# GreatDrake/acg-alp-ldpc

Hardware: AMD Instinct MI355X
Metric: decoded frames/sec (+ FER@SNR) for H05.txt 50-iter BP (higher is better)
Workload: dtype f32; 1 GPU; configs[1]: H05.txt 160x280 E=860 sum-product BP, 50 iterations fixed, 1048576 AWGN frames/GPU/step, HBM-resident; frames_per_gpu=1048576, iters=50, early_exit=False, launcher=single process, engine=fused (messages in LDS)

## Files before the change

acg_alp_ldpc_amd/csrc/api.hip:

```cpp
#include <algorithm>
#include <cmath>
#include <cstdio>
#include <cstdlib>
#include <cstring>

#include "handle.hpp"

namespace acg {

static thread_local std::string g_err;
void set_error(const std::string &msg) { g_err = msg; }
const std::string &last_error() { return g_err; }

bool ScatteredAlloc::create(size_t want, size_t chunk_bytes, int dev, bool shuffle, int spread) {
    hipMemAllocationProp prop{};
    prop.type = hipMemAllocationTypePinned;
    prop.location.type = hipMemLocationTypeDevice;
    prop.location.id = dev;
    size_t gran = 0;
    if (hipMemGetAllocationGranularity(&gran, &prop, hipMemAllocationGranularityMinimum) != hipSuccess || gran == 0) return false;
    chunk = (std::max(chunk_bytes, gran) + gran - 1) / gran * gran;
    const size_t n = (want + chunk - 1) / chunk;
    bytes = n * chunk;
    if (hipMemAddressReserve(&va, bytes, 0, nullptr, 0) != hipSuccess) {
// ... 620 lines not shown
            return 0;
        }
        const int algo_b = (d->p.algo == ACG_LDPC_BP_MINSUM) ? 1 : 0;
        for (int mc = 0; mc < 2; mc++) {
            const bool idxreg = !idxlds && c.max_vdeg <= 4 && lay.n_vpass <= 12 && getenv("ACG_BP_NO_IDXREG") == nullptr;
            const bool regular_b = idxreg && c.max_cdeg <= 8 && c.max_vdeg <= 4 && getenv("ACG_BP_NO_REGULAR") == nullptr && is_regular(c);
            const void *kp = bp_block_kernel_ptr(algo_b, d->f64, L, mc != 0, idxlds, idxreg, regular_b);
            if (mc == 0) {
                d->blk_idxlds = idxlds;
                d->blk_idxreg = idxreg;
            }
            if (!kp) {
                set_error("no workgroup-per-frame kernel instance for this configuration");
                return 3;
            }
            if (int rc = bind_kernel(d, mc, kp)) return rc;
        }
        return 0;
    }
    const int fpw = 64 / L;
    const int waves = wp.waves;
    if (waves == 0) {
        if (d->p.engine == ACG_LDPC_ENGINE_AUTO) {
            d->dev_allocs.clear();
            return decoder_setup_streamed(d);
        }
        set_error("frame state does not fit in LDS (160 KiB per CU)");
        return 3;
    }
    d->block = waves * 64;
    d->frames_per_block = waves * fpw;
    d->lds_block = per_frame * fpw * waves + t.idx_lds_bytes;
    const int algo = (d->p.algo == ACG_LDPC_BP_MINSUM) ? 1 : 0;
    const bool sat = !d->p.early_exit && getenv("ACG_BP_NO_SATSKIP") == nullptr;
    d->phi_memo = sat && getenv("ACG_BP_NO_PHIMEMO") == nullptr;
    d->freeze = sat && algo == 0 && !d->f64 && d->maxd <= 8 && idxlds && llr_regs && getenv("ACG_BP_NO_FREEZE") == nullptr;
    d->freeze_gate = getenv("ACG_BP_FREEZE_NO_GATE") == nullptr;
    d->freeze_first = 10;
    d->freeze_period = 1;
    if (const char *e = getenv("ACG_BP_FREEZE_CADENCE")) {
        int f = 0, q = 0;
        if (sscanf(e, "%d,%d", &f, &q) == 2 && f >= 1 && q >= 1 && f < (1 << 12) && q < (1 << 12)) d->freeze_first = f, d->freeze_period = q;
    }
    d->freeze_slot_words = (size_t) lay.a_words + (size_t) BP_MAX_APASS * L;
    for (int mc = 0; mc < 2; mc++) {
        const int variant = wp.variant;
        d->variant = variant;
        const void *kp = bp_kernel_ptr(algo, d->f64, d->maxd, L, mc != 0, variant, sat);
        if (!kp) {
            set_error("no kernel instance for this configuration");
            return 3;
        }
        if (sat && algo == 0 && !d->f64 && d->maxd <= 8 && variant == 2 && getenv("ACG_BP_NO_SPEC") == nullptr) {
            const char *name = nullptr;
            if (const void *ks = bp_spec_kernel_ptr(lay, mc != 0, &name)) {
                kp = ks;
                d->spec = name;
            }
        }
        if (int rc = bind_kernel(d, mc, kp)) return rc;
    }
    return 0;
}

int acg::acg_ldpc_decoder_create_impl(const acg_ldpc_code *code, const acg_ldpc_params *params, acg_ldpc_decoder **out,
                                      hipStream_t on_stream) {
    if (!code || !params || !out) {
        set_error("null argument");
        return 1;
    }
    if (params->max_iter < 0) {
        set_error("max_iter must be >= 0");
        return 1;
    }
    int ndev = 0;
    if (hipGetDeviceCount(&ndev) != hipSuccess || ndev <= 0) {
        set_error("no HIP device available: libacg_ldpc_hip has no CPU fallback");
        return 20;
    }
    DecoderPtr own(new acg_ldpc_decoder());
    acg_ldpc_decoder *d = own.get();
    d->c = code->c;
    d->p = *params;
    int dev = params->device;
    if (dev < 0) {
        if (hipGetDevice(&dev) != hipSuccess) dev = 0;
    }
    if (dev >= ndev) {
        set_error("device ordinal out of range");
        return 1;
    }
    d->device = dev;
    int rc = 0;
    do {
        if (hipSetDevice(dev) != hipSuccess) { set_error("hipSetDevice failed"); rc = 10; break; }
        hipDeviceProp_t prop;
        if (hipGetDeviceProperties(&prop, dev) != hipSuccess) { set_error("hipGetDeviceProperties failed"); rc = 10; break; }
        d->cu_count = prop.multiProcessorCount;
        if (on_stream) {
            d->stream = on_stream;
            d->own_stream = false;
        } else if (hipStreamCreateWithFlags(&d->stream, hipStreamNonBlocking) != hipSuccess) { set_error("hipStreamCreate failed"); rc = 10; break; }
        if (d->counters.reserve(sizeof(unsigned long long) * MC_NCOUNTERS) ||
            d->work_ring.reserve(sizeof(unsigned long long) * acg_ldpc_decoder::WORK_RING)) { set_error("hipMalloc failed"); rc = 10; break; }
        {
            bool evok = true;
            for (int k = 0; k < acg_ldpc_decoder::WORK_RING; k++)
                evok = evok && hipEventCreate(&d->ring_ev0[k]) == hipSuccess && hipEventCreate(&d->ring_ev[k]) == hipSuccess;
            if (!evok) { set_error("hipEventCreate failed"); rc = 10; break; }
        }
// ... 49 lines not shown
    if (grid_blocks) *grid_blocks = d->grid_cap[0];
}

static std::string describe(const acg_ldpc_decoder *d) {
    char b[512];
    const char *algo = d->p.algo == ACG_LDPC_QPADMM ? "qpadmm" : (d->p.algo == ACG_LDPC_BP_MINSUM ? "minsum" : "sum-product");
    int slabs = 0, f32 = 0;
    int64_t slab = 0;
    if (d->admm && admm_device_streamed(d->admm.get(), &slabs, &slab, &f32)) {
        snprintf(b, sizeof b, "%s engine=streamed kernel=admm_streamed_kernel<%s> f64=%d slab_bytes=%lld slabs=%d workspace_bytes=%lld "
                               "workspace=hipMalloc mc_grid=per-point",
                 algo, f32 ? "float" : "double", f32 ? 0 : 1, (long long) slab, slabs, (long long) slab * slabs);
    } else if (d->admm) {
        int lds = 0, L = 0, fpb = 0, grid = 0;
        admm_device_layout(d->admm.get(), &lds, &L, &fpb, &grid);
        snprintf(b, sizeof b, "%s engine=lds lanes_per_frame=%d frames_per_block=%d lds_bytes_per_frame=%d grid_cap=%d mc_grid=%s", algo, L, fpb, lds, grid,
                 admm_device_has_grid_kernel(d->admm.get()) ? "single-launch" : "per-point");
    } else if (d->streamed) {
        const size_t slab = (size_t) d->stab.ws_words_per_wave * 4;
        snprintf(b, sizeof b, "%s engine=streamed kernel=%s%s f64=%d slab_bytes=%zu slabs=%d workspace_bytes=%zu workspace_base=%p "
                               "workgroups_per_cu=%d schedule=%s",
                 algo, d->sring ? "bp_streamed_ring_kernel" : "bp_streamed_kernel", d->sring ? (d->sring_nt ? "<NT>" : "<default-policy>") : "",
                 d->f64, slab, d->sgrid, slab * (size_t) d->sgrid, d->sws.va, d->sring ? d->sring_per_cu : 2,
                 !d->sws.plain ? "flooding workspace=mapped-chunks" : "flooding workspace=hipMalloc");
        if (!d->sws_probe_ms.empty()) {
            std::string t = b;
            t += " workspace_spread=" + std::to_string(d->sws_spread) + " workspace_probe_ms=";
            for (size_t i = 0; i < d->sws_probe_ms.size(); i++) {
                char q[32];
                snprintf(q, sizeof q, "%s%.2f", i ? "/" : "", d->sws_probe_ms[i]);
                t += q;
            }
            return t;
        }
    } else if (d->layered_block) {
        snprintf(b, sizeof b, "%s engine=fused kernel=%s lanes_per_frame=%d f64=0 block=%d frames_per_block=1 lds_block=%zu "
                               "grid_cap=%d sets=%d steps=%d largest_set=%d schedule=layered messages=%s",
                 algo, d->layered_wide ? "bp_layered_wide_kernel" : "bp_layered_block_kernel", d->L, d->block, d->lds_block, d->grid_cap[0], d->lbtab.n_sets, d->lbtab.n_steps, d->lblay.width,
                 d->p.precision == ACG_LDPC_PREC_F16 ? "fp16" : "fp32");
    } else {
        snprintf(b, sizeof b, "%s engine=fused kernel=%s lanes_per_frame=%d f64=%d block=%d frames_per_block=%d lds_block=%zu grid_cap=%d "
                               "idx_lds=%d idx_reg=%d schedule=%s",
                 algo, d->layered ? "bp_layered_kernel" : (d->pair ? "bp_pair_kernel" : (d->variant < 0 ? "bp_block_kernel" : "bp_fused_kernel")), d->L, d->f64, d->block,
                 d->frames_per_block, d->lds_block, d->grid_cap[0], d->variant < 0 ? (int) d->blk_idxlds : (d->variant > 0), (int) d->blk_idxreg,
                 d->p.schedule == ACG_LDPC_SCHEDULE_LAYERED ? (d->p.precision == ACG_LDPC_PREC_F16 ? "layered messages=fp16" : "layered messages=fp32")
                                                            : "flooding");
        if (d->variant >= 0 && !d->layered && !d->pair) {
            std::string t = b;
            if (!d->p.early_exit) {
                if (d->freeze) t += " freeze=1 freeze_cadence=" + std::to_string(d->freeze_first) + "," + std::to_string(d->freeze_period) +
                                        " freeze_gate=" + (d->freeze_gate ? "1" : "0");
                else t += " freeze=0";
            }
            t += std::string(" spec=") + (d->spec ? d->spec : "0");
            return t;
        }
    }
    return b;
}

int32_t acg_ldpc_decoder_describe(const acg_ldpc_decoder *d, char *buf, int32_t cap) {
    if (!d) return 0;
    return copy_text(describe(d), buf, cap);
}

}
```

acg_alp_ldpc_amd/csrc/bp_core.inc:

```


template <typename T> struct FpBits;
template <> struct FpBits<float> {
    using U = uint32_t;
    static constexpr U SIGN = 0x80000000u;
    static __device__ __forceinline__ U to(float x) { return __float_as_uint(x); }
    static __device__ __forceinline__ float from(U u) { return __uint_as_float(u); }
};
template <> struct FpBits<double> {
    using U = uint64_t;
    static constexpr U SIGN = 0x8000000000000000ull;
    static __device__ __forceinline__ U to(double x) { return (U) __double_as_longlong(x); }
    static __device__ __forceinline__ double from(U u) { return __longlong_as_double((long long) u); }
};

__device__ __forceinline__ void wave_sync() {
    __builtin_amdgcn_fence(__ATOMIC_RELEASE, "wavefront");
    __builtin_amdgcn_wave_barrier();
    __builtin_amdgcn_fence(__ATOMIC_ACQUIRE, "wavefront");
}

template <int L>
__device__ __forceinline__ void group_sync() {
    if (L <= 64) wave_sync();
// ... 42 lines not shown
    static constexpr double scale = 1.0;
    static __device__ __forceinline__ double phi(double x) { return phi_f(x); }
};

__device__ __forceinline__ void philox4x32_10(uint32_t c0, uint32_t c1, uint32_t c2, uint32_t c3, uint32_t k0,
                                              uint32_t k1, uint32_t out[4]) {
#pragma unroll
    for (int r = 0; r < 10; ++r) {
        const uint32_t hi0 = __umulhi(0xD2511F53u, c0), lo0 = 0xD2511F53u * c0;
        const uint32_t hi1 = __umulhi(0xCD9E8D57u, c2), lo1 = 0xCD9E8D57u * c2;
        const uint32_t n0 = hi1 ^ c1 ^ k0, n2 = hi0 ^ c3 ^ k1;
        c0 = n0;
        c1 = lo1;
        c2 = n2;
        c3 = lo0;
        k0 += 0x9E3779B9u;
        k1 += 0xBB67AE85u;
    }
    out[0] = c0;
    out[1] = c1;
    out[2] = c2;
    out[3] = c3;
}

__device__ __forceinline__ void box_muller(uint32_t a, uint32_t b, float &z0, float &z1) {
    const float u1 = ((float) a + 0.5f) * 2.3283064365386963e-10f;
    const float u2 = (float) (b >> 8) * 5.9604644775390625e-08f;
    const float r = sqrtf(-2.0f * 0.693147180559945309f * __builtin_amdgcn_logf(u1));
    z0 = r * __builtin_amdgcn_cosf(u2);
    z1 = r * __builtin_amdgcn_sinf(u2);
}

typedef const int32_t __attribute__((address_space(4))) *sconst_i32;
__device__ __forceinline__ int sload(const int32_t *p, int i) { return ((sconst_i32) (p))[i]; }

template <typename T, int D, int L, int ALGO, bool SAT = false>
struct BpPass {
    using B = FpBits<T>;
    using U = typename B::U;
    static constexpr U SIGN = B::SIGN;
    static constexpr U ONE = (U) 1;

    static __device__ __forceinline__ T phi_c(T s, U mb, T G) {
        T o = G;
        if (B::to(s) != mb) o = Dom<T>::phi(s);
        return o;
    }
    static __device__ __forceinline__ T phi_c(T s) { return phi_c(s, (U) 0, (T) INFINITY); }
    static __device__ __forceinline__ T phi_v(T ax) {
        T o = (T) 0;
        if (!(ax >= (T) 66)) o = Dom<T>::phi(ax);
        return o;
    }

    static __device__ __forceinline__ U check_sat(T *__restrict__ Ap, int slot, const int *cnt, bool write) {
        T x[D];
#pragma unroll
        for (int j = 0; j < D; ++j) x[j] = Ap[j * L];
        U S = 0;
#pragma unroll
        for (int j = 0; j < D; ++j) S ^= B::to(x[j]);
        T mag[D], pre[D], es[D];
        T s = 0;
#pragma unroll
        for (int j = 0; j < D; ++j) {
            mag[j] = B::from(B::to(x[j]) & ~SIGN & ~ONE);
            pre[j] = s;
            s += mag[j];
        }
        T suf = 0;
#pragma unroll
        for (int j = D - 1; j >= 0; --j) {
            es[j] = pre[j] + suf;
            suf += mag[j];
        }
#pragma unroll
        for (int j = 0; j < D; ++j) {
            if (write && slot < cnt[j + 1]) {
                const T o = phi_c(es[j]);
                Ap[j * L] = B::from((B::to(o) & ~SIGN) | ((S ^ B::to(x[j])) & SIGN));
            }
        }
        return S;
    }

    static __device__ __forceinline__ U syn(const T *__restrict__ Ap) {
        T x[D];
#pragma unroll
        for (int j = 0; j < D; ++j) x[j] = Ap[j * L];
        U S = 0;
#pragma unroll
        for (int j = 0; j < D; ++j) S ^= B::to(x[j]);
        return S;
    }

    static __device__ __forceinline__ U syn_abs(const T *__restrict__ Ap, U aw) {
        T x[D];
#pragma unroll
        for (int j = 0; j < D - 1; ++j) x[j] = Ap[j * L];
        U S = aw;
#pragma unroll
        for (int j = 0; j < D - 1; ++j) S ^= B::to(x[j]);
        return S;
    }

    template <bool UNI = false>
    static __device__ __forceinline__ U check(T *__restrict__ Ap, int slot, const int *cnt, bool write, T ms_scale) {
        if constexpr (SAT && ALGO == 0 && !UNI) return check_sat(Ap, slot, cnt, write);
        T x[D];
#pragma unroll
        for (int j = 0; j < D; ++j) x[j] = Ap[j * L];
        U S = 0;
#pragma unroll
        for (int j = 0; j < D; ++j) S ^= B::to(x[j]);
        T out[D];
        if (ALGO == 0) {
            T mag[D], pre[D];
            T s = 0;
#pragma unroll
            for (int j = 0; j < D; ++j) {
                mag[j] = B::from(B::to(x[j]) & ~SIGN & ~ONE);
                pre[j] = s;
                s += mag[j];
            }
            T suf = 0;
#pragma unroll
            for (int j = D - 1; j >= 0; --j) {
                out[j] = Dom<T>::phi(pre[j] + suf);
                suf += mag[j];
            }
        } else {
            T m1 = (T) INFINITY, m2 = (T) INFINITY;
            T mag[D];
#pragma unroll
            for (int j = 0; j < D; ++j) {
                const T a0 = B::from(B::to(x[j]) & ~SIGN & ~ONE);
                const T a = (UNI || slot < cnt[j + 1]) ? a0 : (T) INFINITY;
                mag[j] = a;
                if constexpr (sizeof(T) == 4) m2 = __builtin_amdgcn_fmed3f(a, m1, m2);
                else m2 = __builtin_fmin(m2, __builtin_fmax(a, m1));
                m1 = (sizeof(T) == 4) ? (T) __builtin_fminf((float) m1, (float) a) : (T) __builtin_fmin((double) m1, (double) a);
            }
            const T m1s = ms_scale * m1, m2s = ms_scale * m2;
#pragma unroll
            for (int j = 0; j < D; ++j) out[j] = (mag[j] == m1) ? m2s : m1s;
        }
        if (UNI) {
            U obv[D];
#pragma unroll
            for (int j = 0; j < D; ++j) obv[j] = (B::to(out[j]) & ~SIGN) | ((S ^ B::to(x[j])) & SIGN);
            if (write && slot < cnt[D]) {
#pragma unroll
                for (int j = 0; j < D; ++j) Ap[j * L] = B::from(obv[j]);
            }
            return S;
        }
#pragma unroll
        for (int j = 0; j < D; ++j) {
            const U ob = (B::to(out[j]) & ~SIGN) | ((S ^ B::to(x[j])) & SIGN);
            if (write && slot < cnt[j + 1]) Ap[j * L] = B::from(ob);
        }
        return S;
    }

    static __device__ __forceinline__ U check_abs(T *__restrict__ Ap, int slot, const int *cnt, bool write, U &aw, T allr, T &r_out,
                                                  T ag = (T) INFINITY, U am = 0) {
        T x[D];
#pragma unroll
        for (int j = 0; j < D - 1; ++j) x[j] = Ap[j * L];
        x[D - 1] = B::from(aw);
        U S = 0;
#pragma unroll
        for (int j = 0; j < D; ++j) S ^= B::to(x[j]);
        T out[D];
        T mag[D], pre[D];
        T s = 0;
#pragma unroll
        for (int j = 0; j < D; ++j) {
            mag[j] = B::from(B::to(x[j]) & ~SIGN & ~ONE);
            pre[j] = s;
            s += mag[j];
        }
        T suf = 0;
        if constexpr (SAT) {
#pragma unroll
            for (int j = D - 1; j >= 0; --j) {
                out[j] = pre[j] + suf;
                suf += mag[j];
            }
            const U mb = aw & am;
#pragma unroll
            for (int j = 0; j < D - 1; ++j) {
                if (write && slot < cnt[j + 2]) {
                    const T o = phi_c(out[j], mb, ag);
                    Ap[j * L] = B::from((B::to(o) & ~SIGN) | ((S ^ B::to(x[j])) & SIGN));
                }
            }
            if (write && slot < cnt[1]) {
                const T R = B::from((B::to(phi_c(out[D - 1])) & ~SIGN) | ((S ^ aw) & SIGN));
                r_out = R;
                aw = (aw & ~ONE) | ((allr + R <= (T) 0) ? ONE : (U) 0);
            }
            return S;
        }
#pragma unroll
        for (int j = D - 1; j >= 0; --j) {
            out[j] = Dom<T>::phi(pre[j] + suf);
            suf += mag[j];
        }
#pragma unroll
        for (int j = 0; j < D - 1; ++j) {
            const U ob = (B::to(out[j]) & ~SIGN) | ((S ^ B::to(x[j])) & SIGN);
            if (write && slot < cnt[j + 2]) Ap[j * L] = B::from(ob);
        }
        if (write && slot < cnt[1]) {
            const T R = B::from((B::to(out[D - 1]) & ~SIGN) | ((S ^ aw) & SIGN));
            r_out = R;
            aw = (aw & ~ONE) | ((allr + R <= (T) 0) ? ONE : (U) 0);
        }
        return S;
    }

    template <bool BYTES>
    static __device__ __forceinline__ T &at(T *__restrict__ A, int pos) {
        return BYTES ? *reinterpret_cast<T *>(reinterpret_cast<unsigned char *>(A) + pos) : A[pos];
    }
    template <typename IdxPtr, bool BYTES = false>
    static __device__ __forceinline__ U var(T *__restrict__ A, IdxPtr ip, T llr, int slot, const int *cnt, bool write) {
        int pos[D];
#pragma unroll
        for (int k = 0; k < D; ++k) pos[k] = ip[k * L];
        return var_at<false, BYTES>(A, pos, llr, slot, cnt, write);
    }

    template <bool UNI = false, bool BYTES = false>
    static __device__ __forceinline__ U var_at(T *__restrict__ A, const int (&pos)[D], T llr, int slot, const int *cnt, bool write) {
        T c[D];
#pragma unroll
        for (int k = 0; k < D; ++k) c[k] = at<BYTES>(A, pos[k]);
        T pre[D];
        T s = 0;
#pragma unroll
        for (int k = 0; k < D; ++k) {
            pre[k] = s;
            s += c[k];
        }
        const T total = llr + s;
        const U hard = (total <= (T) 0) ? ONE : (U) 0;
        const U hard_neg = hard | SIGN;
        T suf = 0;
        if constexpr (SAT && ALGO == 0 && !UNI) {
            T xs[D];
#pragma unroll
            for (int k = D - 1; k >= 0; --k) {
                xs[k] = llr + (pre[k] + suf);
                suf += c[k];
            }
#pragma unroll
            for (int k = 0; k < D; ++k) {
                if (write && slot < cnt[k + 1]) {
                    const T mg = phi_v(B::from(B::to(xs[k]) & ~SIGN));
                    at<BYTES>(A, pos[k]) = B::from((B::to(mg) & ~SIGN & ~ONE) | ((xs[k] <= (T) 0) ? hard_neg : hard));
                }
            }
            return hard;
        }
        U ob[D];
#pragma unroll
        for (int k = D - 1; k >= 0; --k) {
            const T xk = llr + (pre[k] + suf);
            suf += c[k];
            const T ax = B::from(B::to(xk) & ~SIGN);
            const T mg = (ALGO == 0) ? Dom<T>::phi(ax) : ax;
            ob[k] = (B::to(mg) & ~SIGN & ~ONE) | ((xk <= (T) 0) ? hard_neg : hard);
        }
        if (UNI) {
            if (write && slot < cnt[D]) {
#pragma unroll
                for (int k = 0; k < D; ++k) at<BYTES>(A, pos[k]) = B::from(ob[k]);
            }
            return hard;
        }
#pragma unroll
        for (int k = 0; k < D; ++k)
            if (write && slot < cnt[k + 1]) at<BYTES>(A, pos[k]) = B::from(ob[k]);
        return hard;
    }

    template <typename IdxPtr, bool BYTES = false>
    static __device__ __forceinline__ void var_init(T *__restrict__ A, IdxPtr ip, T llr, int slot, const int *cnt, bool write) {
        int pos[D];
#pragma unroll
        for (int k = 0; k < D; ++k) pos[k] = ip[k * L];
        const U hard = (llr <= (T) 0) ? ONE : (U) 0;
        const T ax = B::from(B::to(llr) & ~SIGN);
        const T mg = (ALGO == 0) ? Dom<T>::phi(ax) : ax;
        const U ob = (B::to(mg) & ~SIGN & ~ONE) | ((llr <= (T) 0) ? (hard | SIGN) : hard);
#pragma unroll
        for (int k = 0; k < D; ++k)
            if (write && slot < cnt[k + 1]) at<BYTES>(A, pos[k]) = B::from(ob);
    }
};

struct PassRuntime {
    static constexpr bool STATIC = false;
};
#define ACG_PASS_LOOP(ST, p, n, BODY)                                                                          \
    if constexpr (ST) {                                                                                        \
        _Pragma("unroll") for (int p = 0; p < (n); ++p) BODY                                                   \
    } else {                                                                                                   \
        for (int p = 0; p < (n); ++p) BODY                                                                     \
    }

#define ACG_PASS_SWITCH(md, CALL)                                                                              \
    switch (md) {                                                                                              \
        case 1: CALL(1); break;                                                                                \
        case 2: CALL(2); break;                                                                                \
        case 3: CALL(3); break;                                                                                \
        case 4: CALL(4); break;                                                                                \
        case 5: CALL(5); break;                                                                                \
        case 6: CALL(6); break;                                                                                \
        case 7: CALL(7); break;                                                                                \
        case 8: CALL(8); break;                                                                                \
        default: break;                                                                                        \
    }

template <typename T, int MAXD, int L, int ALGO, bool IDXLDS, int NVP, bool IDXB = false, bool SAT = false, typename PS = PassRuntime>
struct BpCore {
    using B = FpBits<T>;
    using U = typename B::U;
    static constexpr U SIGN = B::SIGN;
    static constexpr U ONE = (U) 1;

    const BpTables &t;
    T *__restrict__ A;
    T *__restrict__ LLR;
    uint32_t *__restrict__ OB;
    const uint16_t *IDX;
    const int l;
    const T ms_scale;
    int ccnt[MAXD + 2], vcnt[MAXD + 2];
    using LlrRegs = T[NVP > 0 ? NVP : 1];
    using VarIds = int[NVP > 0 ? NVP : 1];
    static constexpr int NAP = (NVP > 0 && ALGO == 0 && sizeof(T) == 4 && MAXD <= 8 && L <= 64) ? BP_MAX_APASS : 0;
    using AbsLlr = T[NAP > 0 ? NAP : 1];
    using AbsWord = U[NAP > 0 ? NAP : 1];
    __device__ __forceinline__ int n_apass() const {
        if constexpr (PS::STATIC) return NAP > 0 ? PS::n_apass : 0;
        else return NAP > 0 ? t.n_apass : 0;
    }
    static constexpr bool STATIC = PS::STATIC;
    __device__ __forceinline__ int n_cpass() const {
        if constexpr (PS::STATIC) return PS::n_cpass;
        else return t.n_cpass;
    }
    __device__ __forceinline__ int n_vpass() const {
        if constexpr (PS::STATIC) return PS::n_vpass;
        else return t.n_vpass;
// ... 22 lines not shown
        if (NVP > 0) lr[p] = v;
        else LLR[slot] = v;
    }

    __device__ BpCore(const BpTables &t_, T *A_, T *LLR_, uint32_t *OB_, const uint16_t *IDX_, int l_, float s_)
        : t(t_), A(A_), LLR(LLR_), OB(OB_), IDX(IDX_), l(l_), ms_scale((T) s_) {
#pragma unroll
        for (int j = 0; j < MAXD + 2; ++j) {
            if constexpr (PS::STATIC) {
                ccnt[j] = PS::c_cnt_ge(j);
                vcnt[j] = PS::v_cnt_ge(j);
            } else {
                ccnt[j] = sload(t.c_cnt_ge, j);
                vcnt[j] = sload(t.v_cnt_ge, j);
            }
        }
    }

    __device__ __forceinline__ bool syndrome_bad(const AbsWord &aw) const {
        U acc = 0;
        const int nc = n_cpass() - n_apass();
#pragma unroll
        for (int q = 0; q < NAP; ++q) {
            if (q < n_apass()) {
                const int md = c_pass(2 * (nc + q));
                const T *Ap = A + c_pass(2 * (nc + q) + 1) + l;
#define ACG_CALL(D) acc |= BpPass<T, D, L, ALGO>::syn_abs(Ap, aw[q])
                ACG_PASS_SWITCH(md, ACG_CALL)
#undef ACG_CALL
            }
        }
#define ACG_CALL(D) acc |= BpPass<T, D, L, ALGO>::syn(Ap)
#define ACG_BODY                                                       \
    {                                                                  \
        const int md = c_pass(2 * p);                                  \
        const T *Ap = A + c_pass(2 * p + 1) + l;                       \
        if (MAXD <= 8 || md <= 8) {                                    \
            ACG_PASS_SWITCH(md, ACG_CALL)                              \
        } else {                                                       \
            U S = 0;                                                   \
            for (int j = 0; j < md; ++j) S ^= B::to(Ap[j * L]);        \
            acc |= S;                                                  \
        }                                                              \
    }
        ACG_PASS_LOOP(STATIC, p, nc, ACG_BODY)
#undef ACG_BODY
#undef ACG_CALL
        return (acc & ONE) != 0;
    }

    __device__ __forceinline__ U check_phase(bool write, AbsWord &aw, const AbsLlr &al, AbsLlr &ar, const AbsLlr &ag, U am) {
        U acc = 0;
        const int nc = n_cpass() - n_apass();
#define ACG_CALL(D) acc |= BpPass<T, D, L, ALGO, SATSKIP>::check(Ap, slot, ccnt, write, ms_scale)
#define ACG_BODY                                                       \
    {                                                                  \
        const int md = c_pass(2 * p);                                  \
        T *Ap = A + c_pass(2 * p + 1) + l;                             \
        const int slot = p * L + l;                                    \
        if (MAXD <= 8 || md <= 8) {                                    \
            ACG_PASS_SWITCH(md, ACG_CALL)                              \
        } else {                                                       \
            acc |= check_generic(Ap, slot, md, write);                 \
        }                                                              \
    }
        ACG_PASS_LOOP(STATIC, p, nc, ACG_BODY)
#undef ACG_BODY
#undef ACG_CALL
#pragma unroll
        for (int q = 0; q < NAP; ++q) {
            if (q < n_apass()) {
                const int p = nc + q;
                const int md = c_pass(2 * p);
                T *Ap = A + c_pass(2 * p + 1) + l;
                const int slot = p * L + l;
#define ACG_CALL(D) acc |= BpPass<T, D, L, ALGO, SATSKIP>::check_abs(Ap, slot, ccnt, write, aw[q], al[q], ar[q], ag[q], am)
                ACG_PASS_SWITCH(md, ACG_CALL)
#undef ACG_CALL
            }
        }
        return acc;
    }
    __device__ __forceinline__ bool syndrome_bad() const {
        AbsWord aw = {};
        return syndrome_bad(aw);
    }
    __device__ __forceinline__ U check_phase(bool write) {
        AbsWord aw = {};
        AbsLlr al = {}, ar = {}, ag;
#pragma unroll
        for (int q = 0; q < (NAP > 0 ? NAP : 1); ++q) ag[q] = (T) INFINITY;
        return check_phase(write, aw, al, ar, ag, 0);
    }

    __device__ __forceinline__ void var_phase(const LlrRegs &lr, bool write) {
#define ACG_CALL(D) BpPass<T, D, L, ALGO, SATSKIP>::template var<const uint16_t *, IDXB>(A, ip, llr, slot, vcnt, write)
#define ACG_BODY                                                       \
    {                                                                  \
        const int md = v_pass(2 * p);                                  \
        const int ioff = v_pass(2 * p + 1);                            \
        const int slot = p * L + l;                                    \
        const T llr = get_llr(lr, p, slot);                            \
        const uint16_t *ip = IDX + ioff + l;                           \
        if (MAXD <= 8 || md <= 8) {                                    \
            ACG_PASS_SWITCH(md, ACG_CALL)                              \
        } else {                                                       \
            var_generic(ip, llr, slot, md, write);                     \
        }                                                              \
    }
        ACG_PASS_LOOP(STATIC, p, n_vpass(), ACG_BODY)
#undef ACG_BODY
#undef ACG_CALL
    }

    __device__ __forceinline__ uint32_t var_phase_hard(const LlrRegs &lr, bool write) {
        uint32_t hard = 0;
        for (int p = 0; p < t.n_vpass; ++p) {
            const int md = sload(t.v_pass, 2 * p);
            const int ioff = sload(t.v_pass, 2 * p + 1);
            const int slot = p * L + l;
            const T llr = get_llr(lr, p, slot);
            const uint16_t *ip = IDX + ioff + l;
            if (md == 0) {
                hard |= ((llr <= (T) 0) ? 1u : 0u) << p;
            } else if (MAXD <= 8 || md <= 8) {
#define ACG_CALL(D) hard |= (uint32_t) BpPass<T, D, L, ALGO>::template var<const uint16_t *, IDXB>(A, ip, llr, slot, vcnt, write) << p
                ACG_PASS_SWITCH(md, ACG_CALL)
#undef ACG_CALL
            }
        }
        return hard;
    }

    static constexpr int IDXREG_MAXD = 4;
    using IdxRegs = uint32_t[NVP > 0 ? 2 * NVP : 1];
    __device__ __forceinline__ void load_idx_regs(IdxRegs &ir) const {
#pragma unroll
        for (int p = 0; p < (NVP > 0 ? NVP : 0); ++p) {
            uint32_t w[IDXREG_MAXD];
#pragma unroll
            for (int k = 0; k < IDXREG_MAXD; ++k) w[k] = (uint32_t) t.zero_pos;
            if (p < t.n_vpass) {
                const int md = sload(t.v_pass, 2 * p), ioff = sload(t.v_pass, 2 * p + 1);
#pragma unroll
                for (int k = 0; k < IDXREG_MAXD; ++k)
                    if (k < md) w[k] = t.v_apos[ioff + k * L + l];
            }
            ir[2 * p] = w[0] | (w[1] << 16);
            ir[2 * p + 1] = w[2] | (w[3] << 16);
// ... 629 lines not shown
```

acg_alp_ldpc_amd/csrc/bp_inst_spec.hip:

```cpp
#include <hip/hip_runtime.h>

#include "bp_spec.hpp"
#include "launchers.hpp"

namespace acg {
#include "bp_core.inc"

constexpr int BP_NVP = 12;

namespace {
struct BpSpecEntry {
    BpSpecSig sig;
    const void *kernel[2];
};
}

#include "bp_spec_gen.inc"

static const BpSpecEntry spec_entries[] = {ACG_BP_SPEC_ENTRIES {{nullptr, 0, 0, 0, 0, nullptr, nullptr, nullptr, nullptr}, {nullptr, nullptr}}};

const void *bp_spec_kernel_ptr(const BpLayout &lay, bool mc, const char **name) {
    for (const BpSpecEntry *e = spec_entries; e->sig.name; ++e) {
        if (bp_spec_matches(e->sig, lay)) {
            if (name) *name = e->sig.name;
            return e->kernel[mc ? 1 : 0];
        }
    }
    return nullptr;
}

}
```

acg_alp_ldpc_amd/csrc/bp_spec.hpp:

```cpp
#pragma once

#include <cstdint>
#include <vector>

#include "ldpc_internal.hpp"

namespace acg {

constexpr int BP_SPEC_NCNT = 10;

struct BpSpecSig {
    const char *name;
    int L, n_cpass, n_apass, n_vpass;
    const int32_t *c_pass;
    const int32_t *v_pass;
    const int32_t *c_cnt_ge;
    const int32_t *v_cnt_ge;
};

struct BpSpecTables {
    int L = 0, n_cpass = 0, n_apass = 0, n_vpass = 0;
    std::vector<int32_t> c_pass, v_pass, c_cnt_ge, v_cnt_ge;
    BpSpecSig sig(const char *name) const {
        return BpSpecSig{name, L, n_cpass, n_apass, n_vpass, c_pass.data(), v_pass.data(), c_cnt_ge.data(), v_cnt_ge.data()};
    }
};

inline BpSpecTables bp_spec_tables(const BpLayout &lay) {
    BpSpecTables s;
    s.L = lay.L;
    s.n_cpass = lay.n_cpass;
    s.n_apass = lay.n_apass;
    s.n_vpass = lay.n_vpass;
    for (int p = 0; p < lay.n_cpass; p++) {
        s.c_pass.push_back(lay.c_maxdeg[p]);
        s.c_pass.push_back(lay.c_off[p]);
    }
    for (int p = 0; p < lay.n_vpass; p++) {
        s.v_pass.push_back(lay.v_maxdeg[p]);
        s.v_pass.push_back(lay.v_idx_off[p]);
    }
    s.c_cnt_ge.assign(BP_SPEC_NCNT, 0);
    s.v_cnt_ge.assign(BP_SPEC_NCNT, 0);
    for (size_t i = 0; i < lay.c_cnt_ge.size() && i < (size_t) BP_SPEC_NCNT; i++) s.c_cnt_ge[i] = lay.c_cnt_ge[i];
    for (size_t i = 0; i < lay.v_cnt_ge.size() && i < (size_t) BP_SPEC_NCNT; i++) s.v_cnt_ge[i] = lay.v_cnt_ge[i];
    return s;
}

inline bool bp_spec_matches(const BpSpecSig &s, const BpLayout &lay) {
    if (lay.max_cdeg > 8 || lay.max_vdeg > 8) return false;
    if (s.L != lay.L || s.n_cpass != lay.n_cpass || s.n_apass != lay.n_apass || s.n_vpass != lay.n_vpass) return false;
    const BpSpecTables t = bp_spec_tables(lay);
    for (int i = 0; i < 2 * s.n_cpass; i++)
        if (s.c_pass[i] != t.c_pass[i]) return false;
    for (int i = 0; i < 2 * s.n_vpass; i++)
        if (s.v_pass[i] != t.v_pass[i]) return false;
    for (int i = 0; i < BP_SPEC_NCNT; i++)
        if (s.c_cnt_ge[i] != t.c_cnt_ge[i] || s.v_cnt_ge[i] != t.v_cnt_ge[i]) return false;
    return true;
}

}
```

acg_alp_ldpc_amd/csrc/handle.hpp:

```cpp
#pragma once

#include <cstring>
#include <memory>
#include <mutex>
#include <new>

#include "device_mem.hpp"
#include "launchers.hpp"

namespace acg {

const std::string &last_error();

inline int32_t copy_text(const std::string &s, char *buf, int32_t cap) {
    if (buf && cap > 0) {
        const size_t k = std::min<size_t>(s.size(), (size_t) cap - 1);
        std::memcpy(buf, s.data(), k);
        buf[k] = 0;
    }
    return (int32_t) s.size() + 1;
}

template <class F>
int guarded(F &&body) noexcept {
// ... 53 lines not shown
    }
    void release() {
        if (!va) return;
        if (plain) {
            (void) hipFree(va);
            va = nullptr, plain = false;
            return;
        }
        for (size_t i = 0; i < handles.size(); i++) {
            if (mapped[i]) (void) hipMemUnmap((char *) va + i * chunk, chunk);
        }
        for (auto &h : handles) (void) hipMemRelease(h);
        (void) hipMemAddressFree(va, bytes);
        va = nullptr;
        handles.clear();
        mapped.clear();
    }
    bool create(size_t want, size_t chunk_bytes, int dev, bool shuffle, int spread = 1);
};

}

struct acg_ldpc_code {
    acg::Code c;
};

struct acg_ldpc_decoder {
    acg::Code c;
    acg_ldpc_params p;
    int device = 0;
    int cu_count = 256;
    hipStream_t stream = nullptr;
    bool own_stream = true;
    bool ev_valid = false;
    std::recursive_mutex mu;
    std::string name;
    acg::BpLayout lay;
    acg::BpTables tab{};
    std::vector<acg::DeviceBuf> dev_allocs;
    int maxd = 0, f64 = 0, L = 64;
    int block = 256, frames_per_block = 0;
    int grid_cap[2] = {0, 0};
    const void *kernel[2] = {nullptr, nullptr};
    size_t lds_block = 0;
    int variant = -1;
    bool phi_memo = false;
    bool freeze = false;
    bool freeze_count = false;
    bool freeze_gate = true;
    int freeze_first = 0, freeze_period = 0;
    size_t freeze_slot_words = 0;
    acg::DeviceBuf freeze_ws;
    const char *spec = nullptr;
    bool pair = false;
    bool blk_idxlds = false, blk_idxreg = false;
    bool layered = false;
    acg::LayeredLayout llay;
    acg::LayerTables ltab{};
    bool layered_block = false;
    bool layered_wide = false;
    acg::LayeredBlockLayout lblay;
    acg::LayerBlockTables lbtab{};
    acg::DeviceBuf lb_step, lb_pos;
    bool streamed = false;
    acg::StreamTables stab{};
    const void *skernel = nullptr;
    const void *sring = nullptr;
    int sring_per_cu = 2;
    bool sring_nt = false;
    acg::ScatteredAlloc sws;
    std::vector<float> sws_probe_ms;
    int sws_spread = 1;
    int sgrid = 0;
    struct AdmmDrop { void operator()(acg::AdmmDevice *a) const { acg::admm_device_destroy(a); } };
    std::unique_ptr<acg::AdmmDevice, AdmmDrop> admm;
    acg::DeviceBuf st_y, st_bits, st_ok, st_iters;
    std::unique_ptr<acg::HostPipe> pipe;
    acg::DeviceBuf mc_y;
    acg::DeviceBuf cw_dev;
    int64_t cw_count = 0;
    uint64_t cw_hash = 0;
    acg::DeviceBuf counters;
    acg::DeviceBuf det_counters, det_kind, det_sel, det_events, det_words;
    acg::PinnedBuf det_kind_h, det_sel_h, det_counters_h;
    acg::DeviceBuf grid_counters, grid_tab;
    static constexpr int WORK_RING = 32;
    acg::DeviceBuf work_ring;
    hipEvent_t ring_ev0[WORK_RING] = {};
    hipEvent_t ring_ev[WORK_RING] = {};
    bool ring_used[WORK_RING] = {};
    uint64_t launch_seq = 0;
    int last_slot = -1;
    hipStream_t last_stream = nullptr;

    unsigned long long *counters_dev() const { return counters.as<unsigned long long>(); }
    unsigned long long *work_counter(int slot) const { return work_ring.as<unsigned long long>() + slot; }
};

namespace acg {

struct DecoderDrop { void operator()(acg_ldpc_decoder *x) const { acg_ldpc_decoder_destroy(x); } };
using DecoderPtr = std::unique_ptr<acg_ldpc_decoder, DecoderDrop>;

int acg_ldpc_decoder_create_impl(const acg_ldpc_code *code, const acg_ldpc_params *params, acg_ldpc_decoder **out,
                                 hipStream_t on_stream = nullptr);

// ... 15 lines not shown
```

acg_alp_ldpc_amd/csrc/launchers.hpp:

```cpp
#pragma once

#include <hip/hip_runtime.h>

#include <cstdint>
#include <string>
#include <vector>

#include "../../include/acg_ldpc.h"
#include "kernels.hpp"

namespace acg {

struct Code;

const void *bp_kernel_ptr_spa_f32(int maxd, int L, bool mc, int variant, bool sat);
const void *bp_kernel_ptr_spa_f64(int maxd, int L, bool mc, int variant);
const void *bp_kernel_ptr_ms_f32(int maxd, int L, bool mc, int variant);
const void *bp_kernel_ptr_ms_f64(int maxd, int L, bool mc, int variant);
const void *bp_kernel_ptr_spa_f32_dbg(int L);
const void *bp_kernel_ptr_spa_f64_dbg(int L);

struct BpLayout;
const void *bp_spec_kernel_ptr(const BpLayout &lay, bool mc, const char **name);

const void *bp_kernel_ptr(int algo, int f64, int maxd, int L, bool mc, int variant, bool sat);
const void *bp_kernel_ptr_dbg(int f64, int L);
hipError_t bp_launch(const void *kernel, const BpTables &t, const DecodeArgs &a, int grid, int block, size_t lds,
                     hipStream_t s);
hipError_t phi_debug_launch(const void *x, void *out, int n, int f64, hipStream_t s);
hipError_t phi_sat_debug_launch(const float *x, uint32_t *out, int n, hipStream_t s);

hipError_t awgn_launch(float *y, int64_t frames, int n, int nwords, int64_t first_frame, uint64_t seed,
                       const uint32_t *cw_packed, int64_t n_cw, float sigma, hipStream_t s);
hipError_t classify_detail_launch(const float *y, const uint32_t *bits, const uint8_t *ok, const int32_t *iters, int64_t frames,
                                  int n, int nwords, int64_t first_frame, const uint32_t *cw_packed, int64_t n_cw,
                                  unsigned long long *counters, uint8_t *kind, const int32_t *row_ptr, const int32_t *edge_var, int m,
                                  hipStream_t s);
hipError_t gather_events_launch(const int32_t *sel, int n_sel, const float *y, const uint32_t *bits, const uint8_t *ok,
                                const int32_t *iters, const uint8_t *kind, int n, int nwords, int64_t first_frame,
                                const uint32_t *cw_packed, int64_t n_cw, const int32_t *row_ptr, const int32_t *edge_var, int m,
                                acg_ldpc_mc_event *events, uint32_t *words, hipStream_t s);
hipError_t classify_codes_launch(const void *y, int y_is_f64, const uint32_t *bits, const uint8_t *ok, const int32_t *iters,
                                 int64_t frames, int64_t codes, int n, int nwords, int64_t first_frame, const CodeRef *refs, int m,
                                 hipStream_t s);
hipError_t codes_symbols_launch(const double *noise, double *y, int64_t frames, int64_t codes, int n, int nwords, int64_t first_frame,
                                const CodeRef *refs, hipStream_t s);
hipError_t classify_grid_launch(const void *y, int y_is_f64, const uint32_t *bits, const uint8_t *ok, const int32_t *iters,
                                int64_t frames, int64_t points, int n, int nwords, int64_t first_frame, const uint32_t *cw_packed,
                                int64_t n_cw, unsigned long long *counters, const int32_t *row_ptr, const int32_t *edge_var, int m,
                                hipStream_t s);

const void *bp_block_kernel_ptr(int algo, int f64, int L, bool mc, bool idxlds, bool idxreg, bool regular);
const void *bp_block_kernel_ptr_dbg(int f64);
const void *bp_pair_kernel_ptr(int L, bool regular);
const void *bp_layered_kernel_ptr(int G, int waves, bool qc_arith, bool f16, int algo, bool mc);
hipError_t bp_layered_launch(const void *kernel, const LayerTables &t, const DecodeArgs &a, int grid, int block, size_t lds, hipStream_t s);

const void *bp_layered_block_kernel_ptr(int L, bool f16, int algo);
hipError_t bp_layered_block_launch(const void *kernel, const LayerBlockTables &t, const DecodeArgs &a, int grid, int block, size_t lds,
                                   hipStream_t s);

const void *bp_layered_wide_kernel_ptr(int L, bool f16, int algo);
hipError_t bp_layered_wide_launch(const void *kernel, const LayerBlockTables &t, const DecodeArgs &a, int grid, int block, size_t lds,
                                  hipStream_t s);

const void *bp_streamed_ptr(int algo, int f64);
const void *bp_streamed_ring_ptr(int algo, bool nt);
const void *bp_streamed_ring_ptr_dbg();
hipError_t bp_streamed_ring_launch(const void *kernel, const StreamTables &t, const DecodeArgs &a, uint32_t *ws, int grid, hipStream_t s);
hipError_t bp_streamed_launch(const void *kernel, const StreamTables &t, const DecodeArgs &a, uint32_t *ws, int grid,
                              int block, hipStream_t s);

struct AdmmDevice;
AdmmDevice *admm_device_create(const Code &c, const acg_ldpc_params &p, int cu_count, std::string &err);
void admm_device_destroy(AdmmDevice *d);
hipError_t admm_launch(AdmmDevice *d, const DecodeArgs &a, hipStream_t s, std::string &err);
// ... 28 lines not shown
```

Measured before the change: 40.29 million frames/s.

## Add per-row saturation-test masks for specialized BP kernels via host census

Adds a host-side census that simulates BP on sample frames to find which check and variable rows ever hit the saturation or memo cases. It produces per-pass bitmasks so that specialized kernels can drop the saturation branch in rows that never need it and compute phi directly. The runtime PassRuntime path still returns all-ones masks, so the generic kernels behave as before. Only spec kernels whose generated signatures carry sat_rows tables would change, and no such tables appear here. If a mask were derived from the census it could break exactness on inputs the census did not cover.

```diff
diff --git a/acg_alp_ldpc_amd/csrc/api.hip b/acg_alp_ldpc_amd/csrc/api.hip
--- a/acg_alp_ldpc_amd/csrc/api.hip
+++ b/acg_alp_ldpc_amd/csrc/api.hip
@@ -696,10 +696,11 @@
             return 3;
         }
         if (sat && algo == 0 && !d->f64 && d->maxd <= 8 && variant == 2 && getenv("ACG_BP_NO_SPEC") == nullptr) {
-            const char *name = nullptr;
-            if (const void *ks = bp_spec_kernel_ptr(lay, mc != 0, &name)) {
+            const char *name = nullptr, *rows = nullptr;
+            if (const void *ks = bp_spec_kernel_ptr(lay, mc != 0, &name, &rows)) {
                 kp = ks;
                 d->spec = name;
+                d->spec_sat_rows = rows;
             }
         }
         if (int rc = bind_kernel(d, mc, kp)) return rc;
@@ -855,6 +856,7 @@
                                         " freeze_gate=" + (d->freeze_gate ? "1" : "0");
                 else t += " freeze=0";
             }
+            if (d->spec && d->spec_sat_rows) t += std::string(" sat_rows=") + d->spec_sat_rows;
             t += std::string(" spec=") + (d->spec ? d->spec : "0");
             return t;
         }
diff --git a/acg_alp_ldpc_amd/csrc/bp_core.inc b/acg_alp_ldpc_amd/csrc/bp_core.inc
--- a/acg_alp_ldpc_amd/csrc/bp_core.inc
+++ b/acg_alp_ldpc_amd/csrc/bp_core.inc
@@ -118,8 +118,19 @@
         if (!(ax >= (T) 66)) o = Dom<T>::phi(ax);
         return o;
     }
-
-    static __device__ __forceinline__ U check_sat(T *__restrict__ Ap, int slot, const int *cnt, bool write) {
+    static __device__ __forceinline__ U word_c(T s, U mb, T G, U sg, bool test) {
+        if (!test) return (B::to(Dom<T>::phi(s)) & ~SIGN) | sg;
+        U w = (B::to(G) & ~SIGN) | sg;
+        if (B::to(s) != mb) w = (B::to(Dom<T>::phi(s)) & ~SIGN) | sg;
+        return w;
+    }
+    static __device__ __forceinline__ U word_v(T ax, U w, bool test) {
+        if (!test) return w | (B::to(Dom<T>::phi(ax)) & ~SIGN & ~ONE);
+        if (!(ax >= (T) 66)) w |= B::to(Dom<T>::phi(ax)) & ~SIGN & ~ONE;
+        return w;
+    }
+
+    static __device__ __forceinline__ U check_sat(T *__restrict__ Ap, int slot, const int *cnt, bool write, unsigned rows) {
         T x[D];
 #pragma unroll
         for (int j = 0; j < D; ++j) x[j] = Ap[j * L];
@@ -142,10 +153,8 @@
         }
 #pragma unroll
         for (int j = 0; j < D; ++j) {
-            if (write && slot < cnt[j + 1]) {
-                const T o = phi_c(es[j]);
-                Ap[j * L] = B::from((B::to(o) & ~SIGN) | ((S ^ B::to(x[j])) & SIGN));
-            }
+            if (write && slot < cnt[j + 1])
+                Ap[j * L] = B::from(word_c(es[j], (U) 0, (T) INFINITY, (S ^ B::to(x[j])) & SIGN, (rows >> j) & 1u));
         }
         return S;
     }
@@ -171,8 +180,8 @@
     }
 
     template <bool UNI = false>
-    static __device__ __forceinline__ U check(T *__restrict__ Ap, int slot, const int *cnt, bool write, T ms_scale) {
-        if constexpr (SAT && ALGO == 0 && !UNI) return check_sat(Ap, slot, cnt, write);
+    static __device__ __forceinline__ U check(T *__restrict__ Ap, int slot, const int *cnt, bool write, T ms_scale, unsigned rows = ~0u) {
+        if constexpr (SAT && ALGO == 0 && !UNI) return check_sat(Ap, slot, cnt, write, rows);
         T x[D];
 #pragma unroll
         for (int j = 0; j < D; ++j) x[j] = Ap[j * L];
@@ -230,7 +239,7 @@
     }
 
     static __device__ __forceinline__ U check_abs(T *__restrict__ Ap, int slot, const int *cnt, bool write, U &aw, T allr, T &r_out,
-                                                  T ag = (T) INFINITY, U am = 0) {
+                                                  T ag = (T) INFINITY, U am = 0, unsigned rows = ~0u) {
         T x[D];
 #pragma unroll
         for (int j = 0; j < D - 1; ++j) x[j] = Ap[j * L];
@@ -257,13 +266,11 @@
             const U mb = aw & am;
 #pragma unroll
             for (int j = 0; j < D - 1; ++j) {
-                if (write && slot < cnt[j + 2]) {
-                    const T o = phi_c(out[j], mb, ag);
-                    Ap[j * L] = B::from((B::to(o) & ~SIGN) | ((S ^ B::to(x[j])) & SIGN));
-                }
+                if (write && slot < cnt[j + 2])
+                    Ap[j * L] = B::from(word_c(out[j], mb, ag, (S ^ B::to(x[j])) & SIGN, (rows >> j) & 1u));
             }
             if (write && slot < cnt[1]) {
-                const T R = B::from((B::to(phi_c(out[D - 1])) & ~SIGN) | ((S ^ aw) & SIGN));
+                const T R = B::from(word_c(out[D - 1], (U) 0, (T) INFINITY, (S ^ aw) & SIGN, (rows >> (D - 1)) & 1u));
                 r_out = R;
                 aw = (aw & ~ONE) | ((allr + R <= (T) 0) ? ONE : (U) 0);
             }
@@ -292,15 +299,16 @@
         return BYTES ? *reinterpret_cast<T *>(reinterpret_cast<unsigned char *>(A) + pos) : A[pos];
     }
     template <typename IdxPtr, bool BYTES = false>
-    static __device__ __forceinline__ U var(T *__restrict__ A, IdxPtr ip, T llr, int slot, const int *cnt, bool write) {
+    static __device__ __forceinline__ U var(T *__restrict__ A, IdxPtr ip, T llr, int slot, const int *cnt, bool write, unsigned rows = ~0u) {
         int pos[D];
 #pragma unroll
         for (int k = 0; k < D; ++k) pos[k] = ip[k * L];
-        return var_at<false, BYTES>(A, pos, llr, slot, cnt, write);
+        return var_at<false, BYTES>(A, pos, llr, slot, cnt, write, rows);
     }
 
     template <bool UNI = false, bool BYTES = false>
-    static __device__ __forceinline__ U var_at(T *__restrict__ A, const int (&pos)[D], T llr, int slot, const int *cnt, bool write) {
+    static __device__ __forceinline__ U var_at(T *__restrict__ A, const int (&pos)[D], T llr, int slot, const int *cnt, bool write,
+                                               unsigned rows = ~0u) {
         T c[D];
 #pragma unroll
         for (int k = 0; k < D; ++k) c[k] = at<BYTES>(A, pos[k]);
@@ -324,10 +332,8 @@
             }
 #pragma unroll
             for (int k = 0; k < D; ++k) {
-                if (write && slot < cnt[k + 1]) {
-                    const T mg = phi_v(B::from(B::to(xs[k]) & ~SIGN));
-                    at<BYTES>(A, pos[k]) = B::from((B::to(mg) & ~SIGN & ~ONE) | ((xs[k] <= (T) 0) ? hard_neg : hard));
-                }
+                if (write && slot < cnt[k + 1])
+                    at<BYTES>(A, pos[k]) = B::from(word_v(B::from(B::to(xs[k]) & ~SIGN), (xs[k] <= (T) 0) ? hard_neg : hard, (rows >> k) & 1u));
             }
             return hard;
         }
@@ -370,6 +376,8 @@
 
 struct PassRuntime {
     static constexpr bool STATIC = false;
+    static constexpr unsigned c_sat_rows(int) { return ~0u; }
+    static constexpr unsigned v_sat_rows(int) { return ~0u; }
 };
 #define ACG_PASS_LOOP(ST, p, n, BODY)                                                                          \
     if constexpr (ST) {                                                                                        \
@@ -498,7 +506,7 @@
     __device__ __forceinline__ U check_phase(bool write, AbsWord &aw, const AbsLlr &al, AbsLlr &ar, const AbsLlr &ag, U am) {
         U acc = 0;
         const int nc = n_cpass() - n_apass();
-#define ACG_CALL(D) acc |= BpPass<T, D, L, ALGO, SATSKIP>::check(Ap, slot, ccnt, write, ms_scale)
+#define ACG_CALL(D) acc |= BpPass<T, D, L, ALGO, SATSKIP>::check(Ap, slot, ccnt, write, ms_scale, PS::c_sat_rows(p))
 #define ACG_BODY                                                       \
     {                                                                  \
         const int md = c_pass(2 * p);                                  \
@@ -520,7 +528,7 @@
                 const int md = c_pass(2 * p);
                 T *Ap = A + c_pass(2 * p + 1) + l;
                 const int slot = p * L + l;
-#define ACG_CALL(D) acc |= BpPass<T, D, L, ALGO, SATSKIP>::check_abs(Ap, slot, ccnt, write, aw[q], al[q], ar[q], ag[q], am)
+#define ACG_CALL(D) acc |= BpPass<T, D, L, ALGO, SATSKIP>::check_abs(Ap, slot, ccnt, write, aw[q], al[q], ar[q], ag[q], am, PS::c_sat_rows(p))
                 ACG_PASS_SWITCH(md, ACG_CALL)
 #undef ACG_CALL
             }
@@ -540,7 +548,7 @@
     }
 
     __device__ __forceinline__ void var_phase(const LlrRegs &lr, bool write) {
-#define ACG_CALL(D) BpPass<T, D, L, ALGO, SATSKIP>::template var<const uint16_t *, IDXB>(A, ip, llr, slot, vcnt, write)
+#define ACG_CALL(D) BpPass<T, D, L, ALGO, SATSKIP>::template var<const uint16_t *, IDXB>(A, ip, llr, slot, vcnt, write, PS::v_sat_rows(p))
 #define ACG_BODY                                                       \
     {                                                                  \
         const int md = v_pass(2 * p);                                  \
diff --git a/acg_alp_ldpc_amd/csrc/bp_inst_spec.hip b/acg_alp_ldpc_amd/csrc/bp_inst_spec.hip
--- a/acg_alp_ldpc_amd/csrc/bp_inst_spec.hip
+++ b/acg_alp_ldpc_amd/csrc/bp_inst_spec.hip
@@ -19,10 +19,11 @@
 
 static const BpSpecEntry spec_entries[] = {ACG_BP_SPEC_ENTRIES {{nullptr, 0, 0, 0, 0, nullptr, nullptr, nullptr, nullptr}, {nullptr, nullptr}}};
 
-const void *bp_spec_kernel_ptr(const BpLayout &lay, bool mc, const char **name) {
+const void *bp_spec_kernel_ptr(const BpLayout &lay, bool mc, const char **name, const char **sat_rows) {
     for (const BpSpecEntry *e = spec_entries; e->sig.name; ++e) {
         if (bp_spec_matches(e->sig, lay)) {
             if (name) *name = e->sig.name;
+            if (sat_rows) *sat_rows = e->sig.sat_rows;
             return e->kernel[mc ? 1 : 0];
         }
     }
diff --git a/acg_alp_ldpc_amd/csrc/bp_sat_census.hpp b/acg_alp_ldpc_amd/csrc/bp_sat_census.hpp
--- /dev/null
+++ b/acg_alp_ldpc_amd/csrc/bp_sat_census.hpp
@@ -0,0 +1,259 @@
+#pragma once
+
+#include <cmath>
+#include <cstdint>
+#include <cstring>
+#include <random>
+#include <vector>
+
+#include "ldpc_internal.hpp"
+
+namespace acg {
+
+struct SatCensusRow {
+    long units = 0, today = 0, memo = 0, memo_all = 0;
+};
+
+struct SatCensus {
+    std::vector<std::vector<SatCensusRow>> c, v;
+    long frames = 0, fails = 0, sweeps = 0;
+};
+
+namespace sat_census {
+constexpr uint32_t SIGN = 0x80000000u, ONE = 1u;
+inline uint32_t bits(float x) {
+    uint32_t u;
+    memcpy(&u, &x, 4);
+    return u;
+}
+inline float flt(uint32_t u) {
+    float x;
+    memcpy(&x, &u, 4);
+    return x;
+}
+inline float phi(float x) {
+    const float w = x * x;
+    float g = fmaf(w, -1.7256659564749327e-06f, 5.431033644982242e-05f);
+    g = fmaf(g, w, -0.001618721877195048f);
+    g = fmaf(g, w, 0.057762255617977924f);
+    const float ps = fmaf(w, g, 1.5287663729448977f) - log2f(x);
+    const float t = exp2f(-x);
+    const float u = t * t;
+    float r = fmaf(u, 0.40731721508362195f, 0.40423844622223065f);
+    r = fmaf(r, u, 0.5773059513734762f);
+    r = fmaf(r, u, 0.961795680143378f);
+    const float pl = t * fmaf(u, r, 2.8853900817779268f);
+    float o = fmaxf(ps, pl);
+    if (std::isnan(ps) || std::isnan(pl)) o = NAN;
+    return (x >= 66.0f) ? 0.0f : o;
+}
+}
+
+struct SatCensusProbe {
+    virtual void input(int side, int pass, int row, float x) = 0;
+    virtual ~SatCensusProbe() = default;
+};
+
+inline int bp_sat_census_frame(const Code &c, const BpLayout &lay, const float *llr_of_var, int sweeps, bool stop_at_repeat, SatCensus &cs,
+                               std::vector<uint8_t> &est, SatCensusProbe *probe = nullptr) {
+    using namespace sat_census;
+    const int L = lay.L, n = c.n;
+    auto cdeg = [&](int i) { return i < 0 ? 0 : c.row_ptr[i + 1] - c.row_ptr[i]; };
+    auto vdeg = [&](int j) { return j < 0 ? 0 : c.col_ptr[j + 1] - c.col_ptr[j]; };
+    const int nc = lay.n_cpass - lay.n_apass;
+    std::vector<int> d1row((size_t) lay.n_cpass * L, -1);
+    for (int p = 0; p < lay.n_cpass; p++)
+        for (int l = 0; l < L; l++) {
+            const int chk = lay.c_chk[(size_t) p * L + l];
+            if (chk < 0) continue;
+            for (int j = 0; j < cdeg(chk); j++)
+                if (vdeg(c.edge_var[c.row_ptr[chk] + j]) == 1) d1row[(size_t) p * L + l] = p >= nc ? lay.c_maxdeg[p] - 1 : j;
+        }
+    std::vector<uint32_t> A(lay.a_words, 0u);
+    std::vector<float> llr((size_t) lay.n_vpass * L), al((size_t) lay.n_apass * L);
+    std::vector<uint32_t> aw((size_t) lay.n_apass * L), vhard((size_t) lay.n_vpass * L, 0u);
+    for (int p = 0; p < lay.n_vpass; p++)
+        for (int l = 0; l < L; l++) {
+            const int v = lay.v_var[(size_t) p * L + l];
+            const float y = v >= 0 ? llr_of_var[v] : 0.0f;
+            llr[(size_t) p * L + l] = y;
+            const uint32_t hard = y <= 0 ? ONE : 0;
+            vhard[(size_t) p * L + l] = hard;
+            const uint32_t ob = (bits(phi(fabsf(y))) & ~SIGN & ~ONE) | (y <= 0 ? (hard | SIGN) : hard);
+            for (int k = 0; k < vdeg(v); k++) A[lay.v_apos[(size_t) lay.v_idx_off[p] + (size_t) k * L + l]] = ob;
+        }
+    for (int s = 0; s < lay.n_apass * L; s++) {
+        const int v = lay.a_var[s];
+        al[s] = v >= 0 ? llr_of_var[v] : 0.0f;
+        aw[s] = v >= 0 ? (bits(phi(fabsf(al[s]))) & ~SIGN & ~ONE) | (al[s] <= 0 ? (ONE | SIGN) : 0u) : 0u;
+    }
+    constexpr int HIST = 8;
+    std::vector<std::vector<uint32_t>> hist;
+    int run = 0;
+    for (int it = 0; it < sweeps; it++) {
+        for (int p = 0; p < lay.n_cpass; p++) {
+            const int D = lay.c_maxdeg[p];
+            const bool absd = p >= nc;
+            std::vector<char> all_t(D, 1), all_m(D, 1), all_a(D, 1), any(D, 0);
+            for (int l = 0; l < L; l++) {
+                const size_t sl = (size_t) p * L + l;
+                const int chk = lay.c_chk[sl], dg = cdeg(chk);
+                if (chk < 0) continue;
+                uint32_t x[16];
+                for (int j = 0; j < D; j++) x[j] = (absd && j == D - 1) ? aw[sl - (size_t) nc * L] : A[lay.c_off[p] + j * L + l];
+                uint32_t S = 0;
+                for (int j = 0; j < D; j++) S ^= x[j];
+                float mag[16], pre[16], es[16], s = 0, suf = 0;
+                for (int j = 0; j < D; j++) {
+                    mag[j] = flt(x[j] & ~SIGN & ~ONE);
+                    pre[j] = s;
+                    s += mag[j];
+                }
+                for (int j = D - 1; j >= 0; j--) {
+                    es[j] = pre[j] + suf;
+                    suf += mag[j];
+                }
+                const int r1 = d1row[sl];
+                const uint32_t mb = r1 >= 0 ? (x[r1] & ~SIGN & ~ONE) : 0u;
+                for (int j = 0; j < D; j++) {
+                    const bool store = absd ? (j == D - 1 ? dg >= 1 : dg >= j + 2) : dg > j;
+                    if (!store) continue;
+                    any[j] = 1;
+                    if (probe) probe->input(0, p, j, es[j]);
+                    const uint32_t e = bits(es[j]);
+                    const bool t = e == 0;
+                    const bool memo_here = r1 >= 0 && j != r1;
+                    all_t[j] &= t;
+                    all_m[j] &= t || (absd && memo_here && e == mb);
+                    all_a[j] &= t || (memo_here && e == mb);
+                    const float o = t ? INFINITY : phi(es[j]);
+                    if (absd && j == D - 1) {
+                        const float R = flt((bits(o) & ~SIGN) | ((S ^ x[j]) & SIGN));
+                        uint32_t &w = aw[sl - (size_t) nc * L];
+                        w = (w & ~ONE) | ((al[sl - (size_t) nc * L] + R <= 0.0f) ? ONE : 0u);
+                    } else {
+                        A[lay.c_off[p] + j * L + l] = (bits(o) & ~SIGN) | ((S ^ x[j]) & SIGN);
+                    }
+                }
+            }
+            for (int j = 0; j < D; j++)
+                if (any[j]) {
+                    SatCensusRow &r = cs.c[p][j];
+                    r.units++;
+                    r.today += all_t[j];
+                    r.memo += all_m[j];
+                    r.memo_all += all_a[j];
+                }
+        }
+        for (int p = 0; p < lay.n_vpass; p++) {
+            const int D = lay.v_maxdeg[p];
+            std::vector<char> all_v(D, 1), any(D, 0);
+            for (int l = 0; l < L; l++) {
+                const size_t sl = (size_t) p * L + l;
+                const int v = lay.v_var[sl], dg = vdeg(v);
+                if (v < 0) continue;
+                int pos[16];
+                float cv[16], pre[16], s = 0, suf = 0, xs[16];
+                for (int k = 0; k < D; k++) {
+                    pos[k] = lay.v_apos[(size_t) lay.v_idx_off[p] + (size_t) k * L + l];
+                    cv[k] = flt(A[pos[k]]);
+                }
+                for (int k = 0; k < D; k++) {
+                    pre[k] = s;
+                    s += cv[k];
+                }
+                const float y = llr[sl];
+                const uint32_t hard = (y + s <= 0.0f) ? ONE : 0u;
+                vhard[sl] = hard;
+                for (int k = D - 1; k >= 0; k--) {
+                    xs[k] = y + (pre[k] + suf);
+                    suf += cv[k];
+                }
+                for (int k = 0; k < dg; k++) {
+                    any[k] = 1;
+                    const float ax = fabsf(xs[k]);
+                    if (probe) probe->input(1, p, k, ax);
+                    all_v[k] &= ax >= 66.0f;
+                    A[pos[k]] = (bits(phi(ax)) & ~SIGN & ~ONE) | (xs[k] <= 0 ? (hard | SIGN) : hard);
+                }
+            }
+            for (int k = 0; k < D; k++)
+                if (any[k]) {
+                    SatCensusRow &r = cs.v[p][k];
+                    r.units++;
+                    r.today += all_v[k];
+                    r.memo += all_v[k];
+                    r.memo_all += all_v[k];
+                }
+        }
+        run = it + 1;
+        if (stop_at_repeat) {
+            std::vector<uint32_t> st(A);
+            st.insert(st.end(), aw.begin(), aw.end());
+            bool seen = false;
+            for (const auto &h : hist) seen |= h == st;
+            if (seen) break;
+            if ((int) hist.size() == HIST) hist.erase(hist.begin());
+            hist.push_back(std::move(st));
+        }
+    }
+    est.assign(n, 0);
+    for (size_t s = 0; s < vhard.size(); s++)
+        if (lay.v_var[s] >= 0) est[lay.v_var[s]] = (uint8_t) vhard[s];
+    for (size_t s = 0; s < aw.size(); s++)
+        if (lay.a_var[s] >= 0) est[lay.a_var[s]] = (uint8_t) (aw[s] & ONE);
+    return run;
+}
+
+inline SatCensus bp_sat_census_empty(const BpLayout &lay) {
+    SatCensus cs;
+    cs.c.resize(lay.n_cpass);
+    cs.v.resize(lay.n_vpass);
+    for (int p = 0; p < lay.n_cpass; p++) cs.c[p].resize(lay.c_maxdeg[p]);
+    for (int p = 0; p < lay.n_vpass; p++) cs.v[p].resize(lay.v_maxdeg[p]);
+    return cs;
+}
+
+inline SatCensus bp_sat_census(const Code &c, const BpLayout &lay, int frames, int sweeps, double snr, bool stop_at_repeat) {
+    SatCensus cs = bp_sat_census_empty(lay);
+    const double var = std::pow(10, -(snr / 10)) / 2, inv_var2 = 2.0 / var, sigma = std::sqrt(var);
+    std::vector<float> ch(c.n);
+    std::vector<uint8_t> est;
+    for (int f = 0; f < frames; f++) {
+        std::mt19937 rng((uint32_t) (f + 1));
+        std::normal_distribution<double> nd(0.0, 1.0);
+        for (int v = 0; v < c.n; v++) ch[v] = (float) ((1.0 + sigma * nd(rng)) * (inv_var2 * 1.44269504088896341));
+        cs.sweeps += bp_sat_census_frame(c, lay, ch.data(), sweeps, stop_at_repeat, cs, est);
+        bool bad = false;
+        for (int i = 0; i < c.m && !bad; i++) {
+            int x = 0;
+            for (int e = c.row_ptr[i]; e < c.row_ptr[i + 1]; e++) x ^= est[c.edge_var[e]];
+            bad = x != 0;
+        }
+        cs.fails += bad;
+        cs.frames++;
+    }
+    return cs;
+}
+
+inline double bp_sat_share(const SatCensusRow &r) { return r.units ? 100.0 * (double) r.memo / (double) r.units : 0.0; }
+
+struct SatRows {
+    std::vector<uint32_t> c, v;
+};
+inline SatRows bp_sat_rows(const SatCensus &cs, double threshold_pct) {
+    SatRows m;
+    auto side = [&](const std::vector<std::vector<SatCensusRow>> &rows, std::vector<uint32_t> &out) {
+        for (const auto &pass : rows) {
+            uint32_t bitsv = ~0u;
+            for (size_t j = 0; j < pass.size(); j++)
+                if (threshold_pct > 0 && bp_sat_share(pass[j]) < threshold_pct) bitsv &= ~(1u << j);
+            out.push_back(bitsv);
+        }
+    };
+    side(cs.c, m.c);
+    side(cs.v, m.v);
+    return m;
+}
+
+}
diff --git a/acg_alp_ldpc_amd/csrc/bp_spec.hpp b/acg_alp_ldpc_amd/csrc/bp_spec.hpp
--- a/acg_alp_ldpc_amd/csrc/bp_spec.hpp
+++ b/acg_alp_ldpc_amd/csrc/bp_spec.hpp
@@ -16,6 +16,7 @@
     const int32_t *v_pass;
     const int32_t *c_cnt_ge;
     const int32_t *v_cnt_ge;
+    const char *sat_rows = nullptr;
 };
 
 struct BpSpecTables {
diff --git a/acg_alp_ldpc_amd/csrc/handle.hpp b/acg_alp_ldpc_amd/csrc/handle.hpp
--- a/acg_alp_ldpc_amd/csrc/handle.hpp
+++ b/acg_alp_ldpc_amd/csrc/handle.hpp
@@ -129,6 +129,7 @@
     size_t freeze_slot_words = 0;
     acg::DeviceBuf freeze_ws;
     const char *spec = nullptr;
+    const char *spec_sat_rows = nullptr;
     bool pair = false;
     bool blk_idxlds = false, blk_idxreg = false;
     bool layered = false;
diff --git a/acg_alp_ldpc_amd/csrc/launchers.hpp b/acg_alp_ldpc_amd/csrc/launchers.hpp
--- a/acg_alp_ldpc_amd/csrc/launchers.hpp
+++ b/acg_alp_ldpc_amd/csrc/launchers.hpp
@@ -21,7 +21,7 @@
 const void *bp_kernel_ptr_spa_f64_dbg(int L);
 
 struct BpLayout;
-const void *bp_spec_kernel_ptr(const BpLayout &lay, bool mc, const char **name);
+const void *bp_spec_kernel_ptr(const BpLayout &lay, bool mc, const char **name, const char **sat_rows = nullptr);
 
 const void *bp_kernel_ptr(int algo, int f64, int maxd, int L, bool mc, int variant, bool sat);
 const void *bp_kernel_ptr_dbg(int f64, int L);
```

New measurement: 41.21 million frames/s, median of 6. 2.3% higher.
